# torognes/swarm

Hardware: AMD Instinct MI355X
Metric: amplicons/sec clustered (d=1) (higher is better)
Workload: dtype u64; 1 GPU; 10000000 synthetic amplicons x 150 bp, d=1 (10000000 per GPU; the metric's own size; configs[1]: configs1); per_gpu_queries=10000000, db_amplicons=10000000, step=swa_d1_index_build + swa_d1_network_device (B1 seam), db and CSR resident in HBM, route=streaming (d1_stream.inc), build=local, neighbour_links=17077441

## Files before the change

### swarm_amd/csrc/d1.hip

```cpp
#include "d1_internal.h"
using namespace swa_d1;

#include <algorithm>
#include <type_traits>
#include <cstdlib>

namespace {

constexpr size_t kMaxZobristLds = SWA_MAX_ZOBRIST_LDS;

#include "wave_ops.inc"
#include "key_ops.inc"
#include "d1_common.inc"

template <bool ZLDS>
__global__ __launch_bounds__(256) void k_seqhash(const uint64_t * __restrict__ seqs,
                                                 const uint64_t * __restrict__ seq_off,
                                                 const uint32_t * __restrict__ seqlen,
                                                 const uint64_t * __restrict__ zobrist, uint32_t zlen,
                                                 uint32_t n, uint64_t * __restrict__ seqhash,
                                                 swa_aux * __restrict__ aux, uint32_t anchor_w, const uint8_t * __restrict__ only) {
  extern __shared__ uint64_t lds[];
  const uint64_t * zob = zobrist;
  if (ZLDS) {
// ... 406 lines not shown
  g.over = static_cast<uint8_t *>(ctx->d_stream[kSbOver].ptr);
  swa_t0(ctx, kTimeGroups);
  {
    if (!ctx->g1_lds_opt_in) {
      SWA_HIP(ctx, hipFuncSetAttribute(reinterpret_cast<const void *>(&k_group1), hipFuncAttributeMaxDynamicSharedMemorySize, (int)kG1LdsBytes));
      ctx->g1_lds_opt_in = true;
    }
    hipLaunchKernelGGL(k_group1, dim3((unsigned)std::min<uint64_t>(buckets, (uint64_t)ctx->num_cus), 2), dim3(kG1Threads), kG1LdsBytes, ctx->stream, g);
  }
  swa_t1(ctx, kTimeGroups);

  FlatScanArgs f{};
  ListArgs la{};
  for (int i = 0; i < 2; ++i) {
    f.v[i] = g.g[i].kind_cnt; f.units[i] = nullptr; f.fixed[i] = (uint64_t)kListsPerIndex * buckets + 1;
    f.partial[i] = j.partial[i]; f.total[i] = reinterpret_cast<uint32_t *>(scal + 10 + i);
    ListIdx & x = la.x[i];
    x.items_tmp = g.g[i].items_tmp; x.bstart = g.g[i].bstart; x.kind_pos = g.g[i].kind_cnt; x.buckets = (uint32_t)buckets;
    x.l.items = static_cast<swa_item *>(ctx->d_aitems[i].ptr);
    x.l.region = regions;
    x.l.counters = st->counters + kCounterBase + (uint32_t)i * kWidthClasses * 8u;
    x.l.pair_big = g.pair_big;
  }
  const dim3 grid_l((unsigned)std::min<uint64_t>((buckets + 3) / 4, (uint64_t)ctx->num_cus * 8), 2);
  if (plan.lists_inline) {
    uint32_t mask = 0;
    for (uint32_t c = 0; c < kWidthClasses; ++c) { if (ctx->up.d1.class_pop[c] != 0) { mask |= ((1u << kListKinds) - 1u) << (c * kListKinds); } }
    for (int i = 0; i < 2; ++i) { la.x[i].list_mask = mask; }
    hipLaunchKernelGGL(k_group_lists<true>, grid_l, dim3(256), 0, ctx->stream, la);
  } else {
    const dim3 grid_k((unsigned)std::min<uint64_t>(((uint64_t)kListsPerIndex * buckets + kFlatChunk) / kFlatChunk, (uint64_t)ctx->num_cus * 8), 2);
    swa_flat_scan(ctx, grid_k, f);
    hipLaunchKernelGGL(k_group_lists<false>, grid_l, dim3(256), 0, ctx->stream, la);
  }
  ctx->ix.lists_form = plan.lists_inline ? 1 : 0;
  SWA_HIP(ctx, hipGetLastError());
  swa_lap(ctx, "groups + work lists");
  ctx->ix.list_regions_items = item_room;
  ctx->ix.anchor_ready = true;
  ctx->ix.stream_index = true;
  ctx->ix.guard_index = true;
  return SWA_OK;
}

#define SWA_PAIR_CASE(KERNEL, P, WW, NN) \
  if (pass == P && width == WW && nwin == NN) { hipLaunchKernelGGL((KERNEL<P, WW, NN>), dim3(grid), dim3(kThreads), 0, ctx->stream, a); return SWA_OK; }
#define SWA_PAIR_WIDTH(KERNEL, WW) \
  SWA_PAIR_CASE(KERNEL, 0, WW, 1) SWA_PAIR_CASE(KERNEL, 1, WW, 1) SWA_PAIR_CASE(KERNEL, 0, WW, 2) SWA_PAIR_CASE(KERNEL, 1, WW, 2)
#define SWA_PAIR_CASES(KERNEL) \
  SWA_PAIR_WIDTH(KERNEL, 5) SWA_PAIR_WIDTH(KERNEL, 8) SWA_PAIR_WIDTH(KERNEL, 15) SWA_PAIR_WIDTH(KERNEL, 21) \
  SWA_PAIR_CASE(KERNEL, 0, 15, 4) SWA_PAIR_CASE(KERNEL, 1, 15, 4) SWA_PAIR_CASE(KERNEL, 0, 21, 4) SWA_PAIR_CASE(KERNEL, 1, 21, 4)
#define SWA_PAIR_CASE_DYN(KERNEL, P, WW, NN) \
  if (pass == P && width == WW && nwin == NN) { \
    const int bytes = (int)PairLayout<WW>::kDynamicBytes; \
    constexpr uint32_t bit_ = 1u << (P + (WW == 21 ? 2 : 0) + (NN == 2 ? 4 : (NN == 4 ? 8 : 0))); \
    if (bytes != 0 && (ctx->pair_lds_opt_in & bit_) == 0u) {      \
      SWA_HIP(ctx, hipFuncSetAttribute(reinterpret_cast<const void *>(&KERNEL<P, WW, NN>), hipFuncAttributeMaxDynamicSharedMemorySize, bytes)); \
      ctx->pair_lds_opt_in |= bit_; \
    } \
    hipLaunchKernelGGL((KERNEL<P, WW, NN>), dim3(grid), dim3(kThreads), (size_t)bytes, ctx->stream, a); return SWA_OK; }
#define SWA_PAIR_WIDTH_DYN(KERNEL, WW) \
  SWA_PAIR_CASE_DYN(KERNEL, 0, WW, 1) SWA_PAIR_CASE_DYN(KERNEL, 1, WW, 1) SWA_PAIR_CASE_DYN(KERNEL, 0, WW, 2) SWA_PAIR_CASE_DYN(KERNEL, 1, WW, 2)
static int launch_group_pairs(swa_ctx * ctx, int pass, int width, int nwin, int grid, const AnchorArgs & a) {
  SWA_PAIR_WIDTH_DYN(k_d1_group_pairs, 5) SWA_PAIR_WIDTH_DYN(k_d1_group_pairs, 8) SWA_PAIR_WIDTH_DYN(k_d1_group_pairs, 15) SWA_PAIR_WIDTH_DYN(k_d1_group_pairs, 21)
  SWA_PAIR_CASE_DYN(k_d1_group_pairs, 0, 15, 4) SWA_PAIR_CASE_DYN(k_d1_group_pairs, 1, 15, 4) SWA_PAIR_CASE_DYN(k_d1_group_pairs, 0, 21, 4) SWA_PAIR_CASE_DYN(k_d1_group_pairs, 1, 21, 4)
  return swa_fail_msg(ctx, SWA_E_ARG, "pair kernels: no kernel for this record / window width");
}
static int launch_pairs_tiled(swa_ctx * ctx, int pass, int width, int nwin, int grid, const AnchorArgs & a) {
  SWA_PAIR_CASES(k_d1_pairs_tiled)
  return swa_fail_msg(ctx, SWA_E_ARG, "pair kernels: no kernel for this record / window width");
}

static int pair_blocks_per_cu(swa_ctx * ctx, uint32_t cls) {
  int & c = ctx->pair_blocks[cls];
  if (c == 0) {
    int nb = 0;
    const hipError_t e = cls == 0 ? hipOccupancyMaxActiveBlocksPerMultiprocessor(&nb, k_d1_group_pairs<0, 5, 1>, kThreads, 0)
                       : cls == 1 ? hipOccupancyMaxActiveBlocksPerMultiprocessor(&nb, k_d1_group_pairs<0, 8, 1>, kThreads, 0)
                       : cls == 2 ? hipOccupancyMaxActiveBlocksPerMultiprocessor(&nb, k_d1_group_pairs<0, 15, 1>, kThreads, PairLayout<15>::kDynamicBytes)
                                  : hipOccupancyMaxActiveBlocksPerMultiprocessor(&nb, k_d1_group_pairs<0, 21, 1>, kThreads, PairLayout<21>::kDynamicBytes);
    c = (e == hipSuccess && nb >= 1) ? std::min(nb, 8) : (cls <= 1u ? 4 : (cls == 2u ? 2 : 1));
  }
  return c;
}

static uint32_t seg_count(const swa_ctx * ctx) { return (uint32_t)ctx->num_cus * 8u * kWaves; }

static int launch_network_anchored(swa_ctx * ctx, int ncb, uint32_t first, uint32_t count) {
  swa_status_block * st = swa_status(ctx);
  uint32_t * acounters = st->counters;
  SWA_TRY(swa_reserve(ctx, ctx->d_afallback, (2ull * count + 16) * sizeof(swa_fallback)));
  ClearList clears{};
  clear_add(clears, st->stats, sizeof(st->stats));
  clear_add(clears, st->guard + kGuardCall, (kGuardKeys - kGuardCall) * sizeof(uint64_t));
  clear_add(clears, acounters, kCounterBase * sizeof(uint32_t));
  clear_add(clears, ctx->d_seg_fill.ptr, 3ull * seg_count(ctx) * sizeof(uint32_t));
  uint32_t shard_bits = 6;
  while (shard_bits > 0 && (1u << shard_bits) > (uint32_t)ctx->num_cus) { --shard_bits; }
  {
    const uint64_t bytes = ((2ull * kWidthClasses) << shard_bits) * kSchedStride * sizeof(uint32_t);
    SWA_TRY(swa_reserve(ctx, ctx->d_stream[kSbSched], bytes));
    clear_add(clears, ctx->d_stream[kSbSched].ptr, bytes);
  }
  SWA_TRY(swa_reserve(ctx, ctx->d_stream[kSbHeavy], csr_heavy_bytes(count)));
  clear_add(clears, ctx->d_stream[kSbHeavy].ptr, sizeof(uint32_t));
  SWA_TRY(swa_clear_launch(ctx, clears));
  const bool zlds = 4ull * ctx->zobrist_len * sizeof(uint64_t) <= kMaxZobristLds;
  const uint32_t maxwords = (ctx->db.longest + 31u) >> 5;
  swa_t0(ctx, kTimeNetwork);
  const bool window_mode = ctx->ix.anchor_a != 0 || ctx->ix.anchor_b != 0;
  uint64_t item_room = 0;
  const ListRegions regions = list_regions(ctx, &item_room);
  if (item_room != ctx->ix.list_regions_items) { return swa_fail_msg(ctx, SWA_E_ARG, "d=1 network: the work lists in place were laid out for another database"); }
  const int nwin = (int)(ctx->ix.anchor_w / 32u);
  for (int pass = 0; pass < 2; ++pass) {
    swa_t0(ctx, kTimePass + pass);
    AnchorArgs a{};
    a.pass = pass;
    a.no_cluster_breaking = ncb;
    a.first = first; a.count = count;
    a.edges = static_cast<uint64_t *>(ctx->d_edges.ptr);
    a.seg_cap = ctx->seg_cap;
    a.seg_fill = static_cast<uint32_t *>(ctx->d_seg_fill.ptr);
    a.minlen = anchor_minlen(ctx);
    a.win_word = ctx->ix.anchor_a / 32u;
    a.win_word_b = ctx->ix.anchor_b / 32u;
    a.window_mode = window_mode ? 1u : 0u;
    a.seg_staged = static_cast<uint32_t *>(ctx->d_seg_fill.ptr) + (uint64_t)(1 + pass) * seg_count(ctx);
    a.guard = reinterpret_cast<unsigned long long *>(st->guard);
    a.flags = st->flags;
    a.shard_bits = shard_bits;
    a.ids = static_cast<const uint32_t *>(ctx->d_stream[kSbMembers + pass].ptr);
    a.lines = static_cast<const uint4 *>(ctx->d_stream[kSbLines].ptr);
    a.line_quads = ctx->up.d1.lines_quads;
    a.pair_items = static_cast<const swa_item *>(ctx->d_aitems[pass].ptr);
    for (uint32_t cls = 0; cls < kWidthClasses; ++cls) {
      if (ctx->up.d1.class_pop[cls] == 0) { continue; }
      const int width = width_words(cls);
      if (nwin == 4 && width < 15) { return swa_fail_msg(ctx, SWA_E_ARG, "pair kernels: 128-nt windows with sequences of 256 nt or less"); }
      const uint32_t pc = (uint32_t)pass * kWidthClasses + cls;
      for (uint32_t k = 0; k <= kPairClasses; ++k) { a.pair_region[k] = regions.at[cls][k]; }
      a.pair_counters = acounters + kCounterBase + pc * 8u;
      a.items = a.pair_items + regions.at[cls][kPairClasses + 1u];
      a.item_count = a.pair_counters + kPairClasses + 1u;
      a.sched_big = acounters + kCounterSchedBig + 2 * pc;
      a.sched_tiled = acounters + kCounterSchedTiled + 2 * pc;
      a.sched_wide = static_cast<uint32_t *>(ctx->d_stream[kSbSched].ptr) + ((uint64_t)pc << shard_bits) * kSchedStride;
      const uint32_t * have = ctx->ix.list_counts_ready ? ctx->ix.list_counts + pc * 8u : nullptr;
      bool any_pairs = have == nullptr;
      for (uint32_t k = 0; k <= kPairClasses && have != nullptr; ++k) { any_pairs = any_pairs || have[k] != 0u; }
      const int pgrid = ctx->num_cus * pair_blocks_per_cu(ctx, cls);
      {
        uint64_t bundles = 0;
        for (uint32_t k = 0; k < kPairClasses && have != nullptr; ++k) { bundles += ((uint64_t)have[k] + (16u >> k) - 1u) >> (4u - k); }
        const uint64_t waves = (uint64_t)pgrid * 4u;
        a.batch = have == nullptr || bundles >= 16u * waves ? 4u : (bundles >= 8u * waves ? 2u : 1u);
      }
      if (any_pairs) { SWA_TRY(launch_group_pairs(ctx, pass, width, nwin, pgrid, a)); }
      if (have == nullptr || have[kPairClasses + 1u] != 0u) { SWA_TRY(launch_pairs_tiled(ctx, pass, width, nwin, ctx->num_cus * (cls <= 1u ? 8 : 4), a)); }
    }
    swa_t1(ctx, kTimePass + pass);
    SWA_HIP(ctx, hipGetLastError());
  }
  const bool use_member_table = ctx->ix.member_index && !ctx->ix.full_index;
  if (ctx->ix.full_index || ctx->ix.member_index) {
    hipLaunchKernelGGL(k_stream_fallback, dim3(swa_grid_for(ctx, count, 256, 8)), dim3(256), 0, ctx->stream, ctx->db.seqlen, first, count,
                       static_cast<const uint8_t *>(ctx->d_stream[kSbOver].ptr), static_cast<swa_fallback *>(ctx->d_afallback.ptr), acounters + kCounterFallback,
                       ctx->owner_rank, ctx->owner_world, ctx->db.seqs, ctx->db.seq_off, anchor_minlen(ctx));
  }
  NetArgs f{};
  f.seqs = ctx->db.seqs; f.seq_off = ctx->db.seq_off; f.seqlen = ctx->db.seqlen; f.abundance = ctx->db.abundance;
  f.zobrist = static_cast<const uint64_t *>(ctx->d_zobrist.ptr);
  f.zlen = ctx->zobrist_len; f.maxwords = maxwords;
  f.table = static_cast<const swa_slot *>(use_member_table ? ctx->d_stream[kSbMTable].ptr : ctx->d_table.ptr);
  f.tmask = (use_member_table ? ctx->ix.mtable_size : ctx->ix.table_size) - 1;
  f.bloom = static_cast<const uint64_t *>(use_member_table ? ctx->d_stream[kSbMBloom].ptr : ctx->d_bloom.ptr);
  f.bmask = (use_member_table ? ctx->ix.mbloom_words : ctx->ix.bloom_words) - 1;
  f.patterns = static_cast<const uint64_t *>(ctx->d_patterns.ptr);
  f.no_cluster_breaking = ncb;
  f.first = first; f.count = count;
  f.edges = static_cast<uint64_t *>(ctx->d_edges.ptr);
  f.seg_cap = ctx->seg_cap;
  f.seg_fill = static_cast<uint32_t *>(ctx->d_seg_fill.ptr);
  f.fallback = static_cast<const swa_fallback *>(ctx->d_afallback.ptr);
  f.fallback_count = acounters + kCounterFallback;
  f.aux = static_cast<const swa_aux *>(ctx->d_aux.ptr);
  f.owner_rank = 0; f.owner_world = 1;
  f.window_mode = window_mode ? 1u : 0u; f.win_word = ctx->ix.anchor_a / 32u; f.anchor_w = ctx->ix.anchor_w;
  const size_t flds = sizeof(uint64_t) * ((zlds ? 4ull * ctx->zobrist_len : 0ull) + 1024ull +
                                          kWaves * ((size_t)(maxwords + 2u) + kQueueCap + kQueueCap / 2));
  const int fgrid = swa_grid_for(ctx, count, kWaves, 8);
  if (!ctx->ix.full_index && !ctx->ix.member_index) {  }
  else if (zlds) { hipLaunchKernelGGL((k_d1_probe<true, 2>), dim3(fgrid), dim3(kThreads), flds, ctx->stream, f); }
  else { hipLaunchKernelGGL((k_d1_probe<false, 2>), dim3(fgrid), dim3(kThreads), flds, ctx->stream, f); }
  swa_t1(ctx, kTimeNetwork);
  SWA_HIP(ctx, hipGetLastError());
  return SWA_OK;
}

int swa_prepare_hashing(swa_ctx * ctx) {
  const uint32_t n = ctx->db.n;
  ctx->zobrist_len = ctx->db.longest + 2;
  SWA_TRY(swa_reserve(ctx, ctx->d_seqhash, uint64_t(n) * sizeof(uint64_t)));
  SWA_TRY(swa_reserve(ctx, ctx->d_aux, uint64_t(n) * sizeof(swa_aux)));
  if (ctx->zobrist_resident != ctx->zobrist_len) {
    std::vector<uint64_t> zob;
    swa_zobrist_table(ctx->zobrist_len, zob);
    SWA_TRY(swa_reserve(ctx, ctx->d_zobrist, zob.size() * sizeof(uint64_t)));
    SWA_HIP(ctx, hipMemcpyAsync(ctx->d_zobrist.ptr, zob.data(), zob.size() * sizeof(uint64_t), hipMemcpyHostToDevice, ctx->stream));
    SWA_HIP(ctx, hipStreamSynchronize(ctx->stream));
    ctx->zobrist_resident = ctx->zobrist_len;
  }
  return SWA_OK;
}

static int launch_seqhash(swa_ctx * ctx, const uint8_t * only = nullptr) {
  const uint32_t n = ctx->db.n;
  const size_t zbytes = 4ull * ctx->zobrist_len * sizeof(uint64_t);
  const bool zlds = zbytes <= kMaxZobristLds;
  swa_t0(ctx, kTimeSeqhash);
  const int hgrid = swa_grid_for(ctx, n, 256, 8);
  if (zlds) {
    hipLaunchKernelGGL(k_seqhash<true>, dim3(hgrid), dim3(256), zbytes, ctx->stream, ctx->db.seqs, ctx->db.seq_off,
                       ctx->db.seqlen, static_cast<const uint64_t *>(ctx->d_zobrist.ptr), ctx->zobrist_len, n,
                       static_cast<uint64_t *>(ctx->d_seqhash.ptr), static_cast<swa_aux *>(ctx->d_aux.ptr), ctx->ix.anchor_w, only);
  } else {
    hipLaunchKernelGGL(k_seqhash<false>, dim3(hgrid), dim3(256), 0, ctx->stream, ctx->db.seqs, ctx->db.seq_off,
                       ctx->db.seqlen, static_cast<const uint64_t *>(ctx->d_zobrist.ptr), ctx->zobrist_len, n,
                       static_cast<uint64_t *>(ctx->d_seqhash.ptr), static_cast<swa_aux *>(ctx->d_aux.ptr), ctx->ix.anchor_w, only);
  }
  SWA_HIP(ctx, hipGetLastError());
  swa_t1(ctx, kTimeSeqhash);
  return SWA_OK;
}

int swa_hash_sequences(swa_ctx * ctx) {
  SWA_TRY(swa_prepare_hashing(ctx));
  return launch_seqhash(ctx);
}

int swa_ensure_full_index(swa_ctx * ctx) {
  if (ctx->ix.full_index) { return SWA_OK; }
  SWA_TRY(swa_reserve(ctx, ctx->d_table, ctx->ix.table_size * sizeof(swa_slot)));
  SWA_TRY(swa_reserve(ctx, ctx->d_bloom, ctx->ix.bloom_words * sizeof(uint64_t)));
  SWA_TRY(swa_hash_sequences(ctx));
  swa_t0(ctx, kTimeTable);
  SWA_TRY(swa_d1_rebuild_table(ctx, nullptr));
  swa_t1(ctx, kTimeTable);
  ctx->ix.full_index = true;
  return SWA_OK;
}

static int choose_anchor_windows(swa_ctx * ctx) {
  ctx->ix.anchor_a = ctx->ix.anchor_b = 0;
  ctx->ix.anchor_w = 32;
  SWA_TRY(ensure_db_lengths(ctx));
  const uint32_t shortest = ctx->up.d1.db_shortest;
  const uint32_t n = ctx->db.n;
  const uint32_t max_nwin = anchor_max_nwin(ctx);
  ctx->ix.anchor_w = 32u * anchor_nwin_for(shortest, 0u, max_nwin);
  if (windows_search_off()) { return SWA_OK; }
  const uint32_t stride = std::max<uint32_t>(1u, n / 65536u);
  const uint32_t samples = (n + stride - 1) / stride;
  const size_t slots = (size_t)2 * kSampleCandidates * kSampleSlots;
  SWA_TRY(swa_reserve(ctx, ctx->d_akeys[0], std::max<size_t>(ctx->d_akeys[0].bytes, slots * sizeof(uint64_t))));
  SWA_TRY(swa_reserve(ctx, ctx->d_acounts[0], std::max<size_t>(ctx->d_acounts[0].bytes, (slots + 16) * sizeof(uint32_t))));
  auto * keys = static_cast<unsigned long long *>(ctx->d_akeys[0].ptr);
  auto * counts = static_cast<uint32_t *>(ctx->d_acounts[0].ptr);
  uint32_t * stats = counts + slots;
  SWA_HIP(ctx, hipMemsetAsync(keys, 0xFF, slots * sizeof(uint64_t), ctx->stream));
  SWA_HIP(ctx, hipMemsetAsync(counts, 0, (slots + 16) * sizeof(uint32_t), ctx->stream));
  hipLaunchKernelGGL(k_anchor_sample, dim3(swa_grid_for(ctx, samples, 256, 8)), dim3(256), 0, ctx->stream, ctx->db.seqs, ctx->db.seq_off,
                     ctx->db.seqlen, n, stride, keys, counts, stats, shortest, max_nwin);
  hipLaunchKernelGGL(k_sample_mass, dim3(swa_grid_for(ctx, slots, 256, 8)), dim3(256), 0, ctx->stream, counts, stride, stats + 4);
  uint32_t host[8] = {};
  SWA_HIP(ctx, hipMemcpyAsync(host, stats, sizeof(host), hipMemcpyDeviceToHost, ctx->stream));
  SWA_HIP(ctx, hipStreamSynchronize(ctx->stream));
  for (uint32_t c = 0; c < kSampleCandidates; ++c) {
    const bool few_short = host[c] <= samples / 64u || c == 0;
    if (host[4 + c] <= samples / 64u && few_short) {
      ctx->ix.anchor_a = ctx->ix.anchor_b = 32u * c;
      ctx->ix.anchor_w = 32u * anchor_nwin_for(shortest, 32u * c, max_nwin);
      return SWA_OK;
    }
    if (!few_short) { break; }
  }
  return SWA_OK;
}

static int ensure_anchor_windows(swa_ctx * ctx) {
  if (!ctx->up.d1.windows_ready) {
    SWA_TRY(choose_anchor_windows(ctx));
    ctx->up.d1.windows_chosen = ctx->ix.anchor_a;
    ctx->up.d1.windows_w = ctx->ix.anchor_w;
    ctx->up.d1.windows_ready = true;
  }
  ctx->ix.anchor_a = ctx->ix.anchor_b = ctx->up.d1.windows_chosen;
  ctx->ix.anchor_w = ctx->up.d1.windows_w;
  return SWA_OK;
}


static int build_member_index(swa_ctx * ctx, uint32_t dup_first, uint32_t dup_count) {
  ctx->ix.member_index = false;
  const uint32_t n = ctx->db.n;
  SWA_TRY(swa_prepare_hashing(ctx));
  SWA_TRY(launch_seqhash(ctx, static_cast<const uint8_t *>(ctx->d_stream[kSbOver].ptr)));
  uint64_t slots = 1024;
  while (slots < 2ull * ctx->ix.over_mass) { slots <<= 1; }
  const uint64_t words = std::max<uint64_t>(slots >> 3, 1);
// ... 552 lines not shown
```

### swarm_amd/csrc/d1_anchor.inc

```

#ifndef SWA_PAIR_WG
#define SWA_PAIR_WG 5
#endif

__device__ __forceinline__ uint32_t anchor_owner(uint64_t mixed, uint32_t world) {
  return (uint32_t)((((mixed >> 24) & 0xFFFFFFull) * world) >> 24);
}

constexpr uint32_t kRoutePerThread = 8;

__global__ __launch_bounds__(256) void k_anchor_route(const uint64_t * __restrict__ seqs, const uint64_t * __restrict__ seq_off,
                                                      const uint32_t * __restrict__ seqlen, uint32_t first, uint32_t count,
                                                      uint32_t world, uint32_t win_a, uint32_t win_b, uint32_t nwin,
                                                      uint32_t * __restrict__ out, uint64_t cap, uint32_t * counts) {
  __shared__ uint32_t hist[2 * kRouteMaxWorld], base[2 * kRouteMaxWorld];
  const uint32_t tile = 256u * kRoutePerThread;
  for (uint32_t t0 = blockIdx.x * tile; t0 < count; t0 += gridDim.x * tile) {
    if (threadIdx.x < 2u * world) { hist[threadIdx.x] = 0u; }
    __syncthreads();
    uint32_t dest[kRoutePerThread][2], place[kRoutePerThread][2];
#pragma unroll
    for (uint32_t k = 0; k < kRoutePerThread; ++k) {
      const uint32_t e = t0 + k * 256u + threadIdx.x;
      dest[k][0] = dest[k][1] = 0xFFFFFFFFu;
// ... 40 lines not shown
__global__ __launch_bounds__(256) void k_db_lengths(const uint32_t * __restrict__ seqlen, uint32_t n, uint32_t * out) {
  __shared__ uint32_t pop[kWidthClasses + 1];
  if (threadIdx.x <= kWidthClasses) { pop[threadIdx.x] = 0u; }
  __syncthreads();
  uint32_t shortest = 0xFFFFFFFFu, mine[kWidthClasses + 1] = {};
  for (uint32_t i = blockIdx.x * blockDim.x + threadIdx.x; i < n; i += gridDim.x * blockDim.x) {
    const uint32_t len = seqlen[i];
    shortest = min(shortest, len);
    const uint32_t c = width_class(len);
#pragma unroll
    for (uint32_t k = 0; k <= kWidthClasses; ++k) { mine[k] += c == k ? 1u : 0u; }
  }
  for (int o = 32; o > 0; o >>= 1) { shortest = min(shortest, (uint32_t)__shfl_xor((int)shortest, o, 64)); }
#pragma unroll
  for (uint32_t k = 0; k <= kWidthClasses; ++k) {
    uint32_t v = mine[k];
    for (int o = 32; o > 0; o >>= 1) { v += (uint32_t)__shfl_xor((int)v, o, 64); }
    if ((threadIdx.x & 63u) == 0u && v != 0u) { atomicAdd(&pop[k], v); }
  }
  if ((threadIdx.x & 63u) == 0u && shortest != 0xFFFFFFFFu) { atomicMax(out, 0xFFFFFFFFu - shortest); }
  __syncthreads();
  if (threadIdx.x <= kWidthClasses && pop[threadIdx.x] != 0u) { atomicAdd(out + 1u + threadIdx.x, pop[threadIdx.x]); }
}
__global__ __launch_bounds__(256) void k_anchor_sample(const uint64_t * __restrict__ seqs, const uint64_t * __restrict__ seq_off,
                                                       const uint32_t * __restrict__ seqlen, uint32_t n, uint32_t stride,
                                                       unsigned long long * keys, uint32_t * counts, uint32_t * too_short,
                                                       uint32_t shortest, uint32_t max_nwin) {
  for (uint32_t k = blockIdx.x * blockDim.x + threadIdx.x; (uint64_t)k * stride < n; k += gridDim.x * blockDim.x) {
    const uint32_t i = k * stride;
    const uint32_t len = seqlen[i];
    const uint64_t * s = seqs + seq_off[i];
    for (uint32_t c = 0; c < kSampleCandidates; ++c) {
      const uint32_t w = 32u * c, nwin = anchor_nwin_for(shortest, w, max_nwin);
      if (len < 2u * w + 2u * kAnchor * nwin + 1u) { atomicAdd(&too_short[c], 1u); continue; }
      for (int which = 0; which < 2; ++which) {
        const uint64_t key = anchor_key(s, len, which, w, w, nwin);
        unsigned long long * tk = keys + (size_t)(2u * c + (uint32_t)which) * kSampleSlots;
        uint32_t * tc = counts + (size_t)(2u * c + (uint32_t)which) * kSampleSlots;
        uint32_t idx = (uint32_t)mix64(key) & (kSampleSlots - 1u);
        for (uint32_t probes = 0; probes < kSampleSlots; ++probes) {
          const unsigned long long old = atomicCAS(&tk[idx], kKeyEmpty, (unsigned long long)key);
          if (old == kKeyEmpty || old == key) { atomicAdd(&tc[idx], 1u); break; }
          idx = (idx + 1u) & (kSampleSlots - 1u);
        }
      }
    }
  }
}

__global__ __launch_bounds__(256) void k_sample_mass(const uint32_t * __restrict__ counts, uint32_t stride, uint32_t * mass) {
  const uint32_t total = 2u * kSampleCandidates * kSampleSlots;
  for (uint32_t i = blockIdx.x * blockDim.x + threadIdx.x; i < total; i += gridDim.x * blockDim.x) {
    const uint32_t c = counts[i];
    if ((uint64_t)c * stride > kGroupCap) { atomicAdd(&mass[i / (2u * kSampleSlots)], c); }
  }
}

struct PairLists {
  swa_item * items;
  ListRegions region;
  uint32_t * counters;
  uint32_t pair_big;
};

__device__ __forceinline__ uint32_t pair_class(uint32_t g) {
  return g <= 4u ? 0u : (g <= 8u ? 1u : (g <= 16u ? 2u : (g <= 32u ? 3u : 4u)));
}

__global__ __launch_bounds__(256) void k_abundance_rank(const uint64_t * __restrict__ abundance, uint32_t n,
                                                        uint32_t * __restrict__ rank, uint32_t * flags,
                                                        uint32_t * __restrict__ tile_last) {
  __shared__ uint32_t wave_max[4];
  const uint32_t lane = threadIdx.x & 63u, wave = threadIdx.x >> 6;
  for (uint32_t base = blockIdx.x * 256u; base < n; base += gridDim.x * 256u) {
    const uint32_t i = base + threadIdx.x;
    const bool have = i < n;
    const uint64_t ab = have ? abundance[i] : 0ull;
    const uint64_t before = (have && i > 0u) ? abundance[i - 1u] : ~0ull;
    if (have && before < ab) { atomicOr(flags + kFlagUnordered, 1u); }
    uint32_t start = (have && before != ab) ? i + 1u : 0u;
#pragma unroll
    for (int d = 1; d < 64; d <<= 1) {
      const uint32_t up = (uint32_t)__shfl_up((int)start, (unsigned)d, 64);
      if ((int)lane >= d) { start = max(start, up); }
    }
    if (lane == 63u) { wave_max[wave] = start; }
    __syncthreads();
    for (uint32_t w = 0; w < wave; ++w) { start = max(start, wave_max[w]); }
    if (have) { rank[i] = start != 0u ? start - 1u : 0xFFFFFFFFu; }
    if (threadIdx.x == 255u) { tile_last[base >> 8] = start; }
    __syncthreads();
  }
}

__global__ __launch_bounds__(256) void k_abundance_rank_carry(uint32_t * tile_last, uint32_t tiles) {
  constexpr uint32_t kPer = 8;
  __shared__ uint32_t wave_max[4];
  const uint32_t lane = threadIdx.x & 63u, wave = threadIdx.x >> 6;
  uint32_t carry = 0;
  for (uint32_t base = 0; base < tiles; base += 256u * kPer) {
    const uint32_t t0 = base + threadIdx.x * kPer;
    uint32_t v[kPer], mine = 0;
#pragma unroll
    for (uint32_t k = 0; k < kPer; ++k) { v[k] = t0 + k < tiles ? tile_last[t0 + k] : 0u; mine = max(mine, v[k]); }
    uint32_t incl = mine;
#pragma unroll
    for (int d = 1; d < 64; d <<= 1) {
      const uint32_t up = (uint32_t)__shfl_up((int)incl, (unsigned)d, 64);
      if ((int)lane >= d) { incl = max(incl, up); }
    }
    if (lane == 63u) { wave_max[wave] = incl; }
    __syncthreads();
    uint32_t before = carry;
    for (uint32_t w = 0; w < wave; ++w) { before = max(before, wave_max[w]); }
    const uint32_t up1 = (uint32_t)__shfl_up((int)incl, 1u, 64);
    uint32_t run = max(before, lane > 0u ? up1 : 0u);
#pragma unroll
    for (uint32_t k = 0; k < kPer; ++k) {
      if (t0 + k < tiles) { tile_last[t0 + k] = run; }
      run = max(run, v[k]);
    }
    carry = max(carry, max(max(wave_max[0], wave_max[1]), max(wave_max[2], wave_max[3])));
    __syncthreads();
  }
}

__global__ __launch_bounds__(256) void k_abundance_rank_fill(uint32_t n, uint32_t * __restrict__ rank, const uint32_t * __restrict__ tile_last) {
  for (uint32_t i = blockIdx.x * blockDim.x + threadIdx.x; i < n; i += gridDim.x * blockDim.x) {
    if (rank[i] == 0xFFFFFFFFu) { rank[i] = tile_last[i >> 8] - 1u; }
  }
}

__device__ __forceinline__ bool identical_sequences(const uint64_t * seqs, const uint64_t * seq_off, uint32_t len,
                                                    uint32_t x, uint32_t y) {
  const uint64_t * p = seqs + seq_off[x];
  const uint64_t * q = seqs + seq_off[y];
  bool same = true;
  for (uint32_t w = 0; w < ((len + 31u) >> 5); ++w) { same = same && (p[w] == q[w]); }
  return same;
}

struct AnchorArgs {
  const swa_item * items;
  const uint32_t * item_count;
  int pass;
  int no_cluster_breaking;
  uint32_t first, count;
  uint64_t * edges;
  uint64_t seg_cap;
  uint32_t * seg_fill;
  uint32_t * sched_big;
  uint32_t * sched_tiled;
  uint32_t batch;
  uint32_t * sched_wide;
  uint32_t shard_bits;
  uint32_t minlen;
  uint32_t win_word;
  uint32_t window_mode;
  const uint32_t * ids;
  const uint4 * lines;
  uint32_t line_quads;
  const swa_item * pair_items;
  uint64_t pair_region[kPairClasses + 1];
  const uint32_t * pair_counters;
  uint32_t win_word_b;
  uint32_t * seg_staged;
  unsigned long long * guard;
  uint32_t * flags;
};


typedef uint4 __attribute__((may_alias)) uint4_alias;
typedef uint64_t __attribute__((may_alias)) u64_alias;

template <int W> struct PairLayout {
  static constexpr uint32_t kMeta = 4 * W;
  static constexpr uint32_t kDwords = (4 * W + 6 + 3) / 4 * 4;
  static constexpr bool kDynamicLds = 256u * kDwords * 4u > 48u * 1024u;
  static constexpr uint32_t kDynamicBytes = kDynamicLds ? 256u * kDwords * 4u : 0u;
};
template <int W> struct PairMember {
  uint32_t w[2 * W], t[2 * W];
  uint32_t pw_lo, pw_hi, id, len, rank, ok;
};

__device__ __forceinline__ uint32_t first_set_bit(uint32_t x) { uint32_t r; asm("v_ffbl_b32 %0, %1" : "=v"(r) : "v"(x)); return r; }
__device__ __forceinline__ uint32_t leading_zero_bits(uint32_t x) { uint32_t r; asm("v_ffbh_u32 %0, %1" : "=v"(r) : "v"(x)); return r; }

template <int W>
__device__ __forceinline__ void pair_fetch_line(const AnchorArgs & a, bool have, uint32_t id, uint32_t & rank, uint32_t & len, uint64_t (&w64)[W]) {
  rank = 0u; len = 0u;
#pragma unroll
  for (int k = 0; k < W; ++k) { w64[k] = 0ull; }
  if (!have) { return; }
  line_fetch<W>(a.lines, a.line_quads, id, w64, len, rank);
}

template <int W, bool FULL = true>
__device__ __forceinline__ void pair_stage_line(const AnchorArgs & a, bool have, uint32_t id, uint32_t rank, uint32_t len, const uint64_t (&w64)[W],
                                                uint32_t * rec, PairMember<W> & m) {
  uint64_t t64[W];
  m.id = id; m.rank = rank; m.len = len;
  const uint32_t sh = have ? 32u * W - m.len : 0u;
  const uint32_t ws = sh >> 5, b = (sh & 31u) << 1;
#pragma unroll
  for (int k = 0; k < W; ++k) {
    const uint64_t below = k > 0 ? w64[k > 0 ? k - 1 : 0] : 0ull;
    t64[k] = b != 0u ? (w64[k] << b) | (below >> (64u - b)) : w64[k];
  }
  if (__ballot(ws != 0u) != 0ull) {
#pragma unroll
    for (int step = 1; step < W; step <<= 1) {
      const bool take = (ws & (uint32_t)step) != 0u;
#pragma unroll
      for (int k = W - 1; k >= 0; --k) {
        const uint64_t from = k >= step ? t64[k >= step ? k - step : 0] : 0ull;
        t64[k] = take ? from : t64[k];
      }
    }
  }
  uint64_t pw = w64[0];
  if (a.win_word != 0u) {
#pragma unroll
    for (int k = 1; k < W; ++k) { pw = a.win_word == (uint32_t)k ? w64[k] : pw; }
  }
  m.pw_lo = (uint32_t)pw; m.pw_hi = (uint32_t)(pw >> 32);
  m.ok = (have && m.id >= a.first && m.id - a.first < a.count && m.len >= a.minlen) ? 1u : 0u;
  u64_alias * r64 = reinterpret_cast<u64_alias *>(rec);
#pragma unroll
  for (int k = 0; k < W; ++k) {
    m.w[2 * k] = (uint32_t)w64[k]; m.w[2 * k + 1] = (uint32_t)(w64[k] >> 32);
    m.t[2 * k] = (uint32_t)t64[k]; m.t[2 * k + 1] = (uint32_t)(t64[k] >> 32);
    if (FULL) { r64[k] = w64[k]; r64[W + k] = t64[k]; }
  }
  if (FULL) {
    r64[2 * W] = pw;
    rec[4 * W + 2] = m.id; rec[4 * W + 3] = m.len; rec[4 * W + 4] = m.rank; rec[4 * W + 5] = m.ok;
  }
}

template <int W, bool FULL = true>
__device__ __forceinline__ void pair_stage(const AnchorArgs & a, bool have, uint64_t index, uint32_t * rec, PairMember<W> & m) {
  uint64_t w64[W];
  uint32_t rank, len;
  const uint32_t id = have ? a.ids[index] : 0u;
  pair_fetch_line<W>(a, have, id, rank, len, w64);
  pair_stage_line<W, FULL>(a, have, id, rank, len, w64, rec, m);
}

typedef uint32_t swa_u32x4 __attribute__((ext_vector_type(4), may_alias));
template <int W>
__device__ __forceinline__ void pair_load_record(const uint32_t * rec, uint32_t (&p)[PairLayout<W>::kDwords]) {
  typedef const volatile __attribute__((address_space(3))) swa_u32x4 * lds_quads;
  lds_quads q = (lds_quads)rec;
#pragma unroll
  for (uint32_t i = 0; i < PairLayout<W>::kDwords / 4u; ++i) {
    const swa_u32x4 v = q[i];
    p[4 * i] = v.x; p[4 * i + 1] = v.y; p[4 * i + 2] = v.z; p[4 * i + 3] = v.w;
  }
}

template <int W>
__device__ __forceinline__ void pair_member_from(const uint32_t * rec, PairMember<W> & m) {
  uint32_t p[PairLayout<W>::kDwords];
  pair_load_record<W>(rec, p);
#pragma unroll
  for (int k = 0; k < 2 * W; ++k) { m.w[k] = p[k]; m.t[k] = p[2 * W + k]; }
  m.pw_lo = p[4 * W]; m.pw_hi = p[4 * W + 1]; m.id = p[4 * W + 2]; m.len = p[4 * W + 3]; m.rank = p[4 * W + 4]; m.ok = p[4 * W + 5];
}

template <int PASS, int W, int NW>
__device__ __forceinline__ bool pair_near(const PairMember<W> & m, const uint32_t (&p)[PairLayout<W>::kDwords], bool ends, bool & identical) {
  uint32_t f = 0xFFFFFFFFu, l = 0xFFFFFFFFu;
  bool ok = true, same;
  if (ends) {
    uint32_t head = 0u, tail = 0u;
#pragma unroll
    for (int k = 0; k < 2 * W; ++k) {
      if (PASS == 0) {
        if (k < 2 * NW) { head |= m.w[k] ^ p[k]; }
        else {
          f = min(f, first_set_bit(m.w[k] ^ p[k]) | (uint32_t)(32 * k));
          l = min(l, leading_zero_bits(m.t[k] ^ p[2 * W + k]) | (uint32_t)(32 * (2 * W - 1 - k)));
        }
      } else {
        if (k < 2 * NW) { f = min(f, first_set_bit(m.w[k] ^ p[k]) | (uint32_t)(32 * k)); }
        if (k >= 2 * W - 2 * NW) { tail |= m.t[k] ^ p[2 * W + k]; }
        else { l = min(l, leading_zero_bits(m.t[k] ^ p[2 * W + k]) | (uint32_t)(32 * (2 * W - 1 - k))); }
      }
    }
    if (PASS == 0) { asm("" : "+v"(head)); } else { asm("" : "+v"(tail)); }
    if (PASS == 1) { ok = tail == 0u; }
    same = PASS == 0 ? head == 0u : f == 0xFFFFFFFFu;
  } else {
#pragma unroll
    for (int k = 0; k < 2 * W; ++k) {
      f = min(f, first_set_bit(m.w[k] ^ p[k]) | (uint32_t)(32 * k));
      l = min(l, leading_zero_bits(m.t[k] ^ p[2 * W + k]) | (uint32_t)(32 * (2 * W - 1 - k)));
    }
    same = m.pw_lo == p[4 * W] && m.pw_hi == p[4 * W + 1];
  }
  const uint32_t plen = p[4 * W + 3];
  const uint32_t n = min(m.len, plen), apart = max(m.len, plen) - n;
  const uint32_t sum = min(f >> 1, n) + min(l >> 1, n);
  const bool near = apart == 0u ? sum + 1u == n : (apart == 1u && sum >= n);
  identical = PASS == 0 && apart == 0u && f == 0xFFFFFFFFu && same;
  return ok && near && (PASS == 0 ? same : !same);
}

template <int NW>
__device__ __forceinline__ bool pair_misfiled(const uint32_t * mine, const uint32_t * first, uint32_t at, int which) {
  uint32_t diff = 0u;
#pragma unroll
  for (int k = 0; k < 2 * NW; ++k) { diff |= mine[at + k] ^ first[at + k]; }
  if (diff == 0u) { return false; }
  uint64_t wa[NW], wb[NW];
#pragma unroll
  for (int k = 0; k < NW; ++k) {
    wa[k] = (uint64_t)mine[at + 2 * k] | ((uint64_t)mine[at + 2 * k + 1] << 32);
    wb[k] = (uint64_t)first[at + 2 * k] | ((uint64_t)first[at + 2 * k + 1] << 32);
  }
  return anchor_key29(wa, NW, which) != anchor_key29(wb, NW, which);
}
template <int PASS, int W, int NW>
__device__ __forceinline__ uint32_t pair_window_at(const AnchorArgs & a) {
  return PASS == 0 ? 2u * a.win_word : 2u * (uint32_t)W + 2u * ((uint32_t)(W - NW) - a.win_word_b);
}

__device__ __forceinline__ void pair_twin(const AnchorArgs & a, uint32_t ida, uint32_t idb) {
  if (ida != idb && ((ida - a.first < a.count) || (idb - a.first < a.count))) { atomicOr(a.flags + kFlagDuplicates, 1u); }
}

__device__ __forceinline__ uint32_t lanes_below(uint64_t mask) {
  return __builtin_amdgcn_mbcnt_hi((uint32_t)(mask >> 32), __builtin_amdgcn_mbcnt_lo((uint32_t)mask, 0u));
}

__device__ __forceinline__ void pair_emit(bool e1, bool e2, uint32_t id, uint32_t pid, unsigned long long * seg, uint32_t cap,
                                          uint32_t & seg_at) {
  const uint64_t m1 = __ballot(e1), m2 = __ballot(e2);
  if ((m1 | m2) == 0ull) { return; }
  const uint32_t n1 = (uint32_t)__popcll(m1);
  const uint32_t at1 = seg_at + lanes_below(m1), at2 = seg_at + n1 + lanes_below(m2);
  if (e1 && at1 < cap) { seg[at1] = ((unsigned long long)id << 32) | pid; }
  if (e2 && at2 < cap) { seg[at2] = ((unsigned long long)pid << 32) | id; }
  seg_at += n1 + (uint32_t)__popcll(m2);
}

template <int PASS, int W, int NW>
__global__ __launch_bounds__(kThreads) void k_d1_pairs_tiled(const AnchorArgs a) {
  constexpr uint32_t RD = PairLayout<W>::kDwords;
  __shared__ __attribute__((aligned(16))) uint32_t row_recs[kSeedsPerItem * RD];
  const uint32_t wave = threadIdx.x >> 6;
  const uint32_t lane = threadIdx.x & 63u;
  const uint32_t nitems = *a.item_count;
  const uint32_t gwave = blockIdx.x * kWaves + wave;
  uint32_t seg_at = a.seg_fill[gwave];
  unsigned long long * const seg = reinterpret_cast<unsigned long long *>(a.edges) + (uint64_t)gwave * a.seg_cap;
  const uint32_t seg_room = (uint32_t)min(a.seg_cap, (uint64_t)0xFFFFFFFFu);
  uint32_t staged_members = a.seg_staged[gwave], misfiled = 0u;
  const uint32_t win_at = pair_window_at<PASS, W, NW>(a);
  const bool ncb = a.no_cluster_breaking != 0;
  const bool ends = a.window_mode == 0u;
  __shared__ uint32_t sh_it;
  uint32_t it = blockIdx.x, it_next = 0;
  while (it < nitems) {
    const swa_item item = a.items[it];
    const uint32_t g = item.size, r = item.chunk & 63u, part = item.chunk >> 6;
    const uint32_t all_tiles = (g + kSeedsPerItem - 1u) / kSeedsPerItem;
    const uint32_t c_first = r + part * kTiledCols;
    const uint32_t tiles = min(all_tiles, c_first + kTiledCols);
    const uint32_t nrow = min(kSeedsPerItem, g - r * kSeedsPerItem);
    if (threadIdx.x < kSeedsPerItem) {
      const bool have = threadIdx.x < nrow;
      PairMember<W> staged;
      pair_stage<W>(a, have, (uint64_t)item.begin + r * kSeedsPerItem + threadIdx.x, row_recs + threadIdx.x * RD, staged);
      if (part == 0u) { staged_members += (uint32_t)__popcll(__ballot(have)); }
    }
    if (threadIdx.x == 0) { it_next = atomicInc(a.sched_tiled, 0xFFFFFFFFu); }
    __syncthreads();
    if (threadIdx.x < nrow && pair_misfiled<NW>(row_recs + threadIdx.x * RD, row_recs, win_at, PASS)) { ++misfiled; }
    auto column_id = [&](uint32_t c2) -> uint32_t {
      const uint32_t col2 = c2 * kSeedsPerItem + lane;
      return (c2 < tiles && col2 < g) ? a.ids[(uint64_t)item.begin + col2] : 0u;
    };
    uint32_t id_here = column_id(c_first + wave), id_next = column_id(c_first + wave + (uint32_t)kWaves);
    uint64_t w64[W];
    uint32_t rank = 0, len = 0;
    if (c_first + wave < tiles) { pair_fetch_line<W>(a, (c_first + wave) * kSeedsPerItem + lane < g, id_here, rank, len, w64); }
    for (uint32_t c = c_first + wave; c < tiles; c += (uint32_t)kWaves) {
      const uint32_t col = c * kSeedsPerItem + lane;
      const bool have = col < g;
      PairMember<W> m;
      pair_stage_line<W, false>(a, have, id_here, rank, len, w64, nullptr, m);
      {
        const uint32_t cn = c + (uint32_t)kWaves;
        id_here = id_next;
        if (cn < tiles) { pair_fetch_line<W>(a, cn * kSeedsPerItem + lane < g, id_here, rank, len, w64); }
        id_next = column_id(cn + (uint32_t)kWaves);
      }
      if (r == 0u && c != 0u && have) {
        const uint32_t off = PASS == 0 ? win_at : win_at - 2u * (uint32_t)W;
        uint32_t mine[2 * NW], first_win[2 * NW];
#pragma unroll
        for (int q = 0; q < 2 * NW; ++q) {
          mine[q] = 0u;
#pragma unroll
          for (int k = 0; k < 2 * W; ++k) { mine[q] = off + (uint32_t)q == (uint32_t)k ? (PASS == 0 ? m.w[k] : m.t[k]) : mine[q]; }
          first_win[q] = row_recs[win_at + q];
        }
        if (pair_misfiled<NW>(mine, first_win, 0u, PASS)) { ++misfiled; }
      }
      for (uint32_t i = 0; i < nrow; ++i) {
        uint32_t p[RD];
        pair_load_record<W>(row_recs + i * RD, p);
        bool twin = false;
        const bool near = have && (c != r || lane > i) && pair_near<PASS, W, NW>(m, p, ends, twin);
        if (PASS == 0 && twin && have && (c != r || lane > i)) { pair_twin(a, m.id, p[4 * W + 2]); }
        const uint32_t pid = p[4 * W + 2], prank = p[4 * W + 4];
        const bool e1 = near && m.ok != 0u && (ncb || m.rank <= prank);
        const bool e2 = near && p[4 * W + 5] != 0u && (ncb || prank <= m.rank);
        pair_emit(e1, e2, m.id, pid, seg, seg_room, seg_at);
      }
    }
    if (threadIdx.x == 0) { sh_it = gridDim.x + it_next; }
    __syncthreads();
    it = sh_it;
  }
  if (lane == 0u) { a.seg_fill[gwave] = seg_at; a.seg_staged[gwave] = staged_members; }
  if (misfiled != 0u) { atomicAdd(a.guard + kGuardMisfiled, (unsigned long long)misfiled); }
}

template <int PASS, int W, int NW>
__global__ __launch_bounds__(kThreads, W == 5 ? SWA_PAIR_WG : 1) void k_d1_group_pairs(const AnchorArgs a) {
  constexpr uint32_t RD = PairLayout<W>::kDwords;
  constexpr bool kDynamic = PairLayout<W>::kDynamicLds;
  __shared__ __attribute__((aligned(16))) uint32_t recs_static[kDynamic ? 4 : kThreads * RD];
  extern __shared__ __attribute__((aligned(16))) uint32_t recs_dynamic[];
  uint32_t * const recs = kDynamic ? recs_dynamic : recs_static;
  const uint32_t wave = (uint32_t)__builtin_amdgcn_readfirstlane((int)(threadIdx.x >> 6));
  const uint32_t lane = threadIdx.x & 63u;
  const uint32_t gwave = blockIdx.x * kWaves + wave;
  uint32_t seg_at = a.seg_fill[gwave];
  unsigned long long * const seg = reinterpret_cast<unsigned long long *>(a.edges) + (uint64_t)gwave * a.seg_cap;
  const uint32_t seg_room = (uint32_t)min(a.seg_cap, (uint64_t)0xFFFFFFFFu);
  uint32_t staged_members = a.seg_staged[gwave], misfiled = 0u;
  const uint32_t win_at = pair_window_at<PASS, W, NW>(a);
  const bool ncb = a.no_cluster_breaking != 0;
  const bool ends = a.window_mode == 0u;

  const uint32_t nbig = a.pair_counters[kPairClasses];
  const swa_item * big = a.pair_items + a.pair_region[kPairClasses];
  __shared__ uint32_t sh_big;
  uint32_t it = blockIdx.x, it_next = 0;
  while (it < nbig) {
    const swa_item item = big[it];
    const uint32_t g = item.size, half = g >> 1;
    {
      const bool have = threadIdx.x < g;
      PairMember<W> staged;
      pair_stage<W>(a, have, (uint64_t)item.begin + threadIdx.x, recs + threadIdx.x * RD, staged);
      staged_members += (uint32_t)__popcll(__ballot(have));
    }
    if (threadIdx.x == 0) { it_next = atomicInc(a.sched_big, 0xFFFFFFFFu); }
    __syncthreads();
    if (threadIdx.x < g && pair_misfiled<NW>(recs + threadIdx.x * RD, recs, win_at, PASS)) { ++misfiled; }
    for (uint32_t mbase = 0; mbase < g; mbase += 64u) {
      const uint32_t mslot = mbase + lane;
      const bool have = mslot < g;
      PairMember<W> m;
      pair_member_from<W>(recs + (have ? mslot : 0u) * RD, m);
      for (uint32_t t = 1u + wave; t <= half; t += (uint32_t)kWaves) {
        const bool active = have && !(2u * t == g && mslot >= half);
        uint32_t pj = mslot + t;
        pj -= pj >= g ? g : 0u;
        pj = have ? pj : 0u;
        uint32_t p[RD];
        pair_load_record<W>(recs + pj * RD, p);
        bool twin = false;
        const bool near = active && pair_near<PASS, W, NW>(m, p, ends, twin);
        if (PASS == 0 && twin && active) { pair_twin(a, m.id, p[4 * W + 2]); }
        const uint32_t pid = p[4 * W + 2], prank = p[4 * W + 4];
        const bool e1 = near && m.ok != 0u && (ncb || m.rank <= prank);
        const bool e2 = near && p[4 * W + 5] != 0u && (ncb || prank <= m.rank);
        pair_emit(e1, e2, m.id, pid, seg, seg_room, seg_at);
      }
    }
    if (threadIdx.x == 0) { sh_big = gridDim.x + it_next; }
    __syncthreads();
    it = sh_big;
  }
  __syncthreads();

  uint32_t upto[kPairClasses], cls_count[kPairClasses];
  uint64_t cls_region[kPairClasses];
  {
    uint32_t acc = 0;
#pragma unroll
    for (uint32_t k = 0; k < kPairClasses; ++k) {
      const uint32_t c = kPairClasses - 1u - k;
      cls_count[k] = a.pair_counters[c];
      cls_region[k] = a.pair_region[c];
      acc += (cls_count[k] + (16u >> c) - 1u) >> (4u - c);
      upto[k] = acc;
    }
  }
  const uint32_t nbundles = upto[kPairClasses - 1u];
  uint32_t * const myrec = recs + (wave * 64u + lane) * RD;
  const uint32_t kBatch = a.batch;
  const uint32_t nshards = 1u << a.shard_bits;
  const uint32_t shard = blockIdx.x & (nshards - 1u);
  uint32_t * const my_sched = a.sched_wide + (uint64_t)shard * kSchedStride;
  const uint32_t shard_waves = ((gridDim.x + nshards - 1u - shard) >> a.shard_bits) * (uint32_t)kWaves;
  uint32_t bi = 0, batch_left = 0;
  const uint32_t fixed_base = ((blockIdx.x >> a.shard_bits) * (uint32_t)kWaves + wave) * kBatch;
  bool fixed_next = true;
  uint32_t visit = 0;
  auto advance = [&]() -> bool {
    if (batch_left == 0u) {
      const uint32_t base = fixed_next ? fixed_base : (shard_waves + lane_value(visit, 0)) * kBatch;
      fixed_next = false;
      bi = (base << a.shard_bits) + shard;
      if (bi >= nbundles) { return false; }
      batch_left = kBatch;
      if (lane == 0u) { visit = atomicInc(my_sched, 0xFFFFFFFFu); }
    } else {
      bi += nshards;
    }
    --batch_left;
    return bi < nbundles;
  };
  auto describe = [&](uint32_t number, uint32_t & shift, swa_item & item) {
    uint32_t k = 0, before = 0;
#pragma unroll
    for (uint32_t q = 0; q + 1u < kPairClasses; ++q) {
      const bool past = number >= upto[q];
      k += past ? 1u : 0u;
      before = past ? upto[q] : before;
    }
    uint32_t count_c = cls_count[0];
    uint64_t region = cls_region[0];
#pragma unroll
    for (uint32_t q = 1; q < kPairClasses; ++q) {
      count_c = k == q ? cls_count[q] : count_c;
      region = k == q ? cls_region[q] : region;
    }
    shift = 2u + (kPairClasses - 1u - k);
    const uint32_t gi = (number - before) * (64u >> shift) + (lane >> shift);
    item = swa_item{0u, 0u, 0u};
    if (gi < count_c) { item = a.pair_items[region + gi]; }
  };
  auto member_id = [&](uint32_t shift, const swa_item & item) -> uint32_t {
    const uint32_t jj = lane & ((1u << shift) - 1u);
    return jj < item.size ? a.ids[(uint64_t)item.begin + jj] : 0u;
  };
  uint32_t shift0 = 0, shift1 = 0, shift2 = 0, id0 = 0, id1 = 0, g0 = 0, g1 = 0;
  swa_item item2{0u, 0u, 0u};
  uint64_t w64[W];
  uint32_t rank = 0, len = 0;
  bool more0 = advance(), more1 = false, more2 = false;
  if (more0) {
    swa_item item0{0u, 0u, 0u}, item1{0u, 0u, 0u};
    describe(bi, shift0, item0);
    more1 = advance();
    if (more1) { describe(bi, shift1, item1); }
    id0 = member_id(shift0, item0); g0 = item0.size;
    more2 = more1 && advance();
    if (more2) { describe(bi, shift2, item2); }
    if (more1) { id1 = member_id(shift1, item1); g1 = item1.size; }
    pair_fetch_line<W>(a, (lane & ((1u << shift0) - 1u)) < g0, id0, rank, len, w64);
  }
  while (more0) {
    const uint32_t shift = shift0, S = 1u << shift;
    const uint32_t sub = lane >> shift, j = lane & (S - 1u);
    const uint32_t g = g0, half = g >> 1;
    const bool have = j < g;
    PairMember<W> m;
    pair_stage_line<W>(a, have, id0, rank, len, w64, myrec, m);
    staged_members += (uint32_t)__popcll(__ballot(have));
    if (more1) { pair_fetch_line<W>(a, (lane & ((1u << shift1) - 1u)) < g1, id1, rank, len, w64); }
    uint32_t id2 = 0;
    if (more2) { id2 = member_id(shift2, item2); }
    const uint32_t g2 = item2.size;
    const bool more3 = more2 && advance();
    uint32_t shift3 = 0;
    swa_item item3{0u, 0u, 0u};
    if (more3) { describe(bi, shift3, item3); }
    __builtin_amdgcn_fence(__ATOMIC_RELEASE, "wavefront");
    __builtin_amdgcn_wave_barrier();
    __builtin_amdgcn_fence(__ATOMIC_ACQUIRE, "wavefront");
    if (have && pair_misfiled<NW>(myrec, recs + (wave * 64u + (sub << shift)) * RD, win_at, PASS)) { ++misfiled; }
    for (uint32_t t = 1u; t <= 32u; ++t) {
      const bool active = have && t <= half && !(2u * t == g && j >= half);
      if (__ballot(active) == 0ull) { break; }
      uint32_t pj = j + t;
      pj -= pj >= g ? g : 0u;
      pj = active ? pj : j;
      const uint32_t pslot = (sub << shift) + pj;
      uint32_t p[RD];
      pair_load_record<W>(recs + (wave * 64u + pslot) * RD, p);
      bool twin = false;
      const bool near = active && pair_near<PASS, W, NW>(m, p, ends, twin);
      if (PASS == 0 && twin && active) { pair_twin(a, m.id, p[4 * W + 2]); }
      const uint32_t pid = p[4 * W + 2], prank = p[4 * W + 4];
      const bool e1 = near && m.ok != 0u && (ncb || m.rank <= prank);
      const bool e2 = near && p[4 * W + 5] != 0u && (ncb || prank <= m.rank);
      pair_emit(e1, e2, m.id, pid, seg, seg_room, seg_at);
    }
    __builtin_amdgcn_fence(__ATOMIC_RELEASE, "wavefront");
    __builtin_amdgcn_wave_barrier();
    __builtin_amdgcn_fence(__ATOMIC_ACQUIRE, "wavefront");
    more0 = more1; shift0 = shift1; id0 = id1; g0 = g1;
    more1 = more2; shift1 = shift2; id1 = id2; g1 = g2;
    more2 = more3; shift2 = shift3; item2 = item3;
  }
  if (lane == 0u) { a.seg_fill[gwave] = seg_at; a.seg_staged[gwave] = staged_members; }
  if (misfiled != 0u) { atomicAdd(a.guard + kGuardMisfiled, (unsigned long long)misfiled); }
}
```

Before: 6.039 billion amplicons/s.

## Process smallest pair groups one-per-lane in registers on a subset of blocks

Adds a lane-per-group path in the group-pairs kernel: groups of size up to 4 (pair class 0) are handled by a single lane each, which loads the members into registers and compares them pairwise without LDS staging or bundle scheduling. Only the first ~40% of blocks run this path, and class 0 is dropped from the bundle count and the host-side batch sizing, so the other blocks handle the larger classes. This is meant to remove the LDS round trips and wave-level bundle overhead for tiny groups. The cost is more register pressure and possible load imbalance between lane blocks and bundle blocks. It is disabled for width 21.

New measurement: 6.012 billion amplicons/s. Within noise of the previous version (-0.4%).

```diff
diff --git a/swarm_amd/csrc/d1.hip b/swarm_amd/csrc/d1.hip
--- a/swarm_amd/csrc/d1.hip
+++ b/swarm_amd/csrc/d1.hip
@@ -582,10 +582,11 @@
       const int pgrid = ctx->num_cus * pair_blocks_per_cu(ctx, cls);
       {
         uint64_t bundles = 0;
-        for (uint32_t k = 0; k < kPairClasses && have != nullptr; ++k) { bundles += ((uint64_t)have[k] + (16u >> k) - 1u) >> (4u - k); }
+        for (uint32_t k = pair_lane_groups(width) ? 1u : 0u; k < kPairClasses && have != nullptr; ++k) { bundles += ((uint64_t)have[k] + (16u >> k) - 1u) >> (4u - k); }
         const uint64_t waves = (uint64_t)pgrid * 4u;
         a.batch = have == nullptr || bundles >= 16u * waves ? 4u : (bundles >= 8u * waves ? 2u : 1u);
       }
+      a.lane_blocks = (uint32_t)std::max(1, pgrid * 2 / 5);
       if (any_pairs) { SWA_TRY(launch_group_pairs(ctx, pass, width, nwin, pgrid, a)); }
       if (have == nullptr || have[kPairClasses + 1u] != 0u) { SWA_TRY(launch_pairs_tiled(ctx, pass, width, nwin, ctx->num_cus * (cls <= 1u ? 8 : 4), a)); }
     }
diff --git a/swarm_amd/csrc/d1_anchor.inc b/swarm_amd/csrc/d1_anchor.inc
--- a/swarm_amd/csrc/d1_anchor.inc
+++ b/swarm_amd/csrc/d1_anchor.inc
@@ -216,6 +216,7 @@
   uint32_t * sched_big;
   uint32_t * sched_tiled;
   uint32_t batch;
+  uint32_t lane_blocks;
   uint32_t * sched_wide;
   uint32_t shard_bits;
   uint32_t minlen;
@@ -243,6 +244,8 @@
   static constexpr bool kDynamicLds = 256u * kDwords * 4u > 48u * 1024u;
   static constexpr uint32_t kDynamicBytes = kDynamicLds ? 256u * kDwords * 4u : 0u;
 };
+template <int W> constexpr bool kPairLaneGroups = W != 21;
+constexpr bool pair_lane_groups(int width) { return width == 5 ? kPairLaneGroups<5> : (width == 8 ? kPairLaneGroups<8> : (width == 15 ? kPairLaneGroups<15> : kPairLaneGroups<21>)); }
 template <int W> struct PairMember {
   uint32_t w[2 * W], t[2 * W];
   uint32_t pw_lo, pw_hi, id, len, rank, ok;
@@ -261,8 +264,8 @@
 }
 
 template <int W, bool FULL = true>
-__device__ __forceinline__ void pair_stage_line(const AnchorArgs & a, bool have, uint32_t id, uint32_t rank, uint32_t len, const uint64_t (&w64)[W],
-                                                uint32_t * rec, PairMember<W> & m) {
+__device__ __forceinline__ void pair_stage_line_at(const AnchorArgs & a, uint32_t win_word, bool have, uint32_t id, uint32_t rank, uint32_t len,
+                                                   const uint64_t (&w64)[W], uint32_t * rec, PairMember<W> & m) {
   uint64_t t64[W];
   m.id = id; m.rank = rank; m.len = len;
   const uint32_t sh = have ? 32u * W - m.len : 0u;
@@ -284,9 +287,9 @@
     }
   }
   uint64_t pw = w64[0];
-  if (a.win_word != 0u) {
-#pragma unroll
-    for (int k = 1; k < W; ++k) { pw = a.win_word == (uint32_t)k ? w64[k] : pw; }
+  if (win_word != 0u) {
+#pragma unroll
+    for (int k = 1; k < W; ++k) { pw = win_word == (uint32_t)k ? w64[k] : pw; }
   }
   m.pw_lo = (uint32_t)pw; m.pw_hi = (uint32_t)(pw >> 32);
   m.ok = (have && m.id >= a.first && m.id - a.first < a.count && m.len >= a.minlen) ? 1u : 0u;
@@ -301,6 +304,12 @@
     r64[2 * W] = pw;
     rec[4 * W + 2] = m.id; rec[4 * W + 3] = m.len; rec[4 * W + 4] = m.rank; rec[4 * W + 5] = m.ok;
   }
+}
+
+template <int W, bool FULL = true>
+__device__ __forceinline__ void pair_stage_line(const AnchorArgs & a, bool have, uint32_t id, uint32_t rank, uint32_t len, const uint64_t (&w64)[W],
+                                                uint32_t * rec, PairMember<W> & m) {
+  pair_stage_line_at<W, FULL>(a, a.win_word, have, id, rank, len, w64, rec, m);
 }
 
 template <int W, bool FULL = true>
@@ -331,6 +340,15 @@
 #pragma unroll
   for (int k = 0; k < 2 * W; ++k) { m.w[k] = p[k]; m.t[k] = p[2 * W + k]; }
   m.pw_lo = p[4 * W]; m.pw_hi = p[4 * W + 1]; m.id = p[4 * W + 2]; m.len = p[4 * W + 3]; m.rank = p[4 * W + 4]; m.ok = p[4 * W + 5];
+}
+
+template <int W>
+__device__ __forceinline__ void pair_record_of(const PairMember<W> & m, uint32_t (&p)[PairLayout<W>::kDwords]) {
+#pragma unroll
+  for (int k = 0; k < 2 * W; ++k) { p[k] = m.w[k]; p[2 * W + k] = m.t[k]; }
+  p[4 * W] = m.pw_lo; p[4 * W + 1] = m.pw_hi; p[4 * W + 2] = m.id; p[4 * W + 3] = m.len; p[4 * W + 4] = m.rank; p[4 * W + 5] = m.ok;
+#pragma unroll
+  for (uint32_t k = 4 * W + 6; k < PairLayout<W>::kDwords; ++k) { p[k] = 0u; }
 }
 
 template <int PASS, int W, int NW>
@@ -389,6 +407,31 @@
 template <int PASS, int W, int NW>
 __device__ __forceinline__ uint32_t pair_window_at(const AnchorArgs & a) {
   return PASS == 0 ? 2u * a.win_word : 2u * (uint32_t)W + 2u * ((uint32_t)(W - NW) - a.win_word_b);
+}
+
+template <int PASS, int W, int NW>
+__device__ __forceinline__ bool pair_misfiled_regs(const PairMember<W> & m, const uint32_t (&first)[PairLayout<W>::kDwords], bool ends, uint32_t win_at) {
+  uint32_t mine[2 * NW], theirs[2 * NW];
+  if (ends) {
+#pragma unroll
+    for (int q = 0; q < 2 * NW; ++q) {
+      mine[q] = PASS == 0 ? m.w[q] : m.t[2 * (W - NW) + q];
+      theirs[q] = first[(PASS == 0 ? 0 : 2 * W + 2 * (W - NW)) + q];
+    }
+    return pair_misfiled<NW>(mine, theirs, 0u, PASS);
+  }
+  const uint32_t off = PASS == 0 ? win_at : win_at - 2u * (uint32_t)W;
+#pragma unroll
+  for (int q = 0; q < 2 * NW; ++q) {
+    mine[q] = 0u; theirs[q] = 0u;
+#pragma unroll
+    for (int k = 0; k < 2 * W; ++k) {
+      const bool here = off + (uint32_t)q == (uint32_t)k;
+      mine[q] = here ? (PASS == 0 ? m.w[k] : m.t[k]) : mine[q];
+      theirs[q] = here ? first[(PASS == 0 ? 0 : 2 * W) + k] : theirs[q];
+    }
+  }
+  return pair_misfiled<NW>(mine, theirs, 0u, PASS);
 }
 
 __device__ __forceinline__ void pair_twin(const AnchorArgs & a, uint32_t ida, uint32_t idb) {
@@ -555,6 +598,76 @@
   }
   __syncthreads();
 
+  if constexpr (kPairLaneGroups<W>) {
+    if (blockIdx.x < a.lane_blocks) {
+      const uint32_t nsmall = a.pair_counters[0];
+      const swa_item * const small = a.pair_items + a.pair_region[0];
+      const uint32_t stride = a.lane_blocks * (uint32_t)kWaves * 64u;
+      auto lane_item = [&](uint32_t at) -> swa_item {
+        swa_item item{0u, 0u, 0u};
+        if (at < nsmall && at + lane < nsmall) { item = small[at + lane]; }
+        return item;
+      };
+      struct Raw { uint64_t w64[W]; uint32_t id, rank, len; };
+      auto lane_member = [&](const swa_item & item, uint32_t j, Raw & r) __attribute__((always_inline)) {
+        r.id = j < item.size ? a.ids[(uint64_t)item.begin + j] : 0u;
+      };
+      auto lane_line = [&](bool have, Raw & r) __attribute__((always_inline)) {
+        pair_fetch_line<W>(a, have, r.id, r.rank, r.len, r.w64);
+        staged_members += (uint32_t)__popcll(__ballot(have));
+      };
+      auto lane_partner = [&](const Raw & r, uint32_t win_word, bool active, uint32_t (&p)[RD]) __attribute__((always_inline)) {
+        PairMember<W> partner;
+        pair_stage_line_at<W, false>(a, win_word, active, r.id, r.rank, r.len, r.w64, nullptr, partner);
+        pair_record_of<W>(partner, p);
+      };
+      auto lane_round = [&](const Raw & r, uint32_t win_word, bool ends_, bool first, bool active, const uint32_t (&p)[RD]) __attribute__((always_inline)) {
+        PairMember<W> m;
+        pair_stage_line_at<W, false>(a, win_word, active, r.id, r.rank, r.len, r.w64, nullptr, m);
+        if (first && active && pair_misfiled_regs<PASS, W, NW>(m, p, ends_, win_at)) { ++misfiled; }
+        bool twin = false;
+        const bool near = active && pair_near<PASS, W, NW>(m, p, ends_, twin);
+        if (PASS == 0 && twin && active) { pair_twin(a, m.id, p[4 * W + 2]); }
+        const uint32_t pid = p[4 * W + 2], prank = p[4 * W + 4];
+        const bool e1 = near && m.ok != 0u && (ncb || m.rank <= prank);
+        const bool e2 = near && p[4 * W + 5] != 0u && (ncb || prank <= m.rank);
+        pair_emit(e1, e2, m.id, pid, seg, seg_room, seg_at);
+      };
+      auto lane_rounds = [&](const Raw & r0, const Raw & r1, const Raw & r2, const Raw & r3, uint32_t g, uint32_t win_word, bool ends_) __attribute__((always_inline)) {
+        if (__ballot(1u < g) != 0ull) {
+          uint32_t p[RD];
+          lane_partner(r1, win_word, 1u < g, p);
+          lane_round(r0, win_word, ends_, true, 1u < g, p);
+        }
+        if (__ballot(2u < g) != 0ull) {
+          uint32_t p[RD];
+          lane_partner(r2, win_word, 2u < g, p);
+          lane_round(r0, win_word, ends_, true, 2u < g, p);
+          lane_round(r1, win_word, ends_, false, 2u < g, p);
+        }
+        if (__ballot(3u < g) != 0ull) {
+          uint32_t p[RD];
+          lane_partner(r3, win_word, 3u < g, p);
+          lane_round(r0, win_word, ends_, true, 3u < g, p);
+          lane_round(r1, win_word, ends_, false, 3u < g, p);
+          lane_round(r2, win_word, ends_, false, 3u < g, p);
+        }
+      };
+      constexpr bool kPrefetch = W != 5;
+      uint32_t base = gwave * 64u;
+      swa_item item = lane_item(base);
+      for (; base < nsmall; base += stride) {
+        const uint32_t g = min(item.size, 4u);
+        Raw r0, r1, r2, r3;
+        lane_member(item, 0u, r0); lane_member(item, 1u, r1); lane_member(item, 2u, r2); lane_member(item, 3u, r3);
+        if (kPrefetch) { item = lane_item(base + stride); }
+        lane_line(0u < g, r0); lane_line(1u < g, r1); lane_line(2u < g, r2); lane_line(3u < g, r3);
+        if (ends) { lane_rounds(r0, r1, r2, r3, g, 0u, true); } else { lane_rounds(r0, r1, r2, r3, g, a.win_word, false); }
+        if (!kPrefetch) { item = lane_item(base + stride); }
+      }
+    }
+  }
+
   uint32_t upto[kPairClasses], cls_count[kPairClasses];
   uint64_t cls_region[kPairClasses];
   {
@@ -564,7 +677,7 @@
       const uint32_t c = kPairClasses - 1u - k;
       cls_count[k] = a.pair_counters[c];
       cls_region[k] = a.pair_region[c];
-      acc += (cls_count[k] + (16u >> c) - 1u) >> (4u - c);
+      acc += (c == 0u && kPairLaneGroups<W>) ? 0u : (cls_count[k] + (16u >> c) - 1u) >> (4u - c);
       upto[k] = acc;
     }
   }
```
